# SerCharles/CN-RMA

Hardware: AMD Instinct MI355X
Metric: scenes/sec fwd (40-view->192^3 voxel): dense unprojection + RMA + voxelise + FCAF3D + decode (higher is better)
Workload: dtype f32 (sparse conv f16x3: 22-bit operands, fp32 accumulate; value_f32_conv = exact fp32); 1 GPU; NS: 40 views x 256 ch x 480x640 fp32 maps (channels_last) -> grid 192x192x192, N=300, max_points=500000, FCAF3D MinkResNet34 + head, 1 HIP graph per scene, 3 in flight; M_rows=72216505, M_selected=500000, M_unique=496819

## Files before the change

cn-rma_amd/csrc/rma.hip:

```cpp
#include "common.h"

#include <stdlib.h>

namespace {

struct MarchParams {
  int V, H, W, X, Y, Z, N;
  float vs, ox, oy, oz, t_one, thr;
};

struct Ray {
  float ox, oy, oz, dx, dy, dz;
};

__device__ __forceinline__ Ray make_ray(const float* __restrict__ Pi, float u, float v) {
  float far_[3], o[3];
#pragma unroll
  for (int r = 0; r < 3; ++r) {
    float acc = Pi[r * 4 + 0] * u;
    acc = fmaf(Pi[r * 4 + 1], v, acc);
    acc = fmaf(Pi[r * 4 + 2], 1.0f, acc);
    acc = fmaf(Pi[r * 4 + 3], 1.0f, acc);
    far_[r] = acc;
    o[r] = Pi[r * 4 + 3];
// ... 81 lines not shown
}

template <typename Keep>
__device__ __forceinline__ void neus_march(const Ray& r, const MarchParams& p, const float* __restrict__ tsdf,
                                           float s_out, Keep keep) {
  int a, b;
  if (!clip_steps(r, p, &a, &b)) return;
  double acc = 1.0;
  Sample cur = eval_step(r, a, p, tsdf);
  for (int n = a; n <= b; ++n) {
    Sample nxt;
    if (n + 1 <= b) {
      nxt = eval_step(r, n + 1, p, tsdf);
    } else {
      nxt = cur;
      if (n + 1 <= p.N - 1) { nxt.s = s_out; nxt.valid = false; }
    }
    float alpha = fmaxf((cur.s - nxt.s) / cur.s, 0.0f);
    float T = (float)acc;
    float w = T * alpha;
    if (cur.valid && w >= p.thr) keep(n, cur, w);
    acc *= (double)(1.0f - alpha);
    if ((float)acc < p.thr) break;
    cur = nxt;
  }
}

__device__ __forceinline__ bool ray_setup(const MarchParams& p, const float* __restrict__ proj_inv, int64_t r, Ray* ray,
                                          int* view, int* pix) {
  const int64_t HW = (int64_t)p.H * p.W;
  if (r >= (int64_t)p.V * HW) return false;
  *view = (int)(r / HW);
  *pix = (int)(r - (int64_t)(*view) * HW);
  int v = *pix / p.W, u = *pix - v * p.W;
  *ray = make_ray(proj_inv + (int64_t)(*view) * 16, (float)u, (float)v);
  return true;
}

struct EmitDst {
  float* xyz; int xyz_stride;
  float* w; int w_stride;
  float* feat; int feat_stride;
  int32_t* sample;
  const int32_t* sel;
  const float* w_div;
  float ax, ay, az;
  int64_t sel_cap = 0;
  int64_t out_cap = 0;
};

__global__ __launch_bounds__(256) void neus_count_kernel(MarchParams p, const float* __restrict__ proj_inv,
                                                         const float* __restrict__ tsdf, int32_t* __restrict__ count,
                                                         double* __restrict__ wsum, int2* __restrict__ kept, int cap,
                                                         int32_t* __restrict__ overflow) {
  const int64_t r = (int64_t)blockIdx.x * blockDim.x + threadIdx.x;
  Ray ray; int view, pix;
  if (!ray_setup(p, proj_inv, r, &ray, &view, &pix)) return;
  const float s_out = sigmoid_neg(1.0f);
  int c = 0;
  double ws = 0.0;
  int2* mine = kept ? kept + r * cap : nullptr;
  neus_march(ray, p, tsdf, s_out, [&](int n, const Sample&, float w) {
    if (mine) {
      if (c < cap) mine[c] = make_int2(__float_as_int(w), n);
      else atomicAdd(overflow, 1);
    }
    ++c;
    ws += (double)w;
  });
  count[r] = c;
  wsum[r] = ws;
}

__device__ __forceinline__ float div_by_vs(float a, float vs, float y) {
  float q = a * y;
  float r = fmaf(-vs, q, a);
  q = fmaf(r, y, q);
  r = fmaf(-vs, q, a);
  return fmaf(r, y, q);
}

struct TabSample { float s; bool valid; int rad; };

constexpr int SKIP_B = 4, SKIP_RMAX = 16;

__device__ __forceinline__ TabSample fetch_step(const Ray& r, int n, const MarchParams& p, float inv_vs,
                                                const float* __restrict__ tab, float s_out,
                                                const uint8_t* __restrict__ skip = nullptr, int by = 0, int bz = 0) {
  const float t = (float)n * p.t_one;
  const float x = r.ox + r.dx * t, y = r.oy + r.dy * t, z = r.oz + r.dz * t;
  const float fx = rintf(div_by_vs(x - p.ox, p.vs, inv_vs));
  const float fy = rintf(div_by_vs(y - p.oy, p.vs, inv_vs));
  const float fz = rintf(div_by_vs(z - p.oz, p.vs, inv_vs));
  TabSample o;
  o.valid = (fx >= 0.0f) && (fx < (float)p.X) && (fy >= 0.0f) && (fy < (float)p.Y) && (fz >= 0.0f) && (fz < (float)p.Z);
  o.s = s_out;
  o.rad = 0;
  if (o.valid) {
    o.s = tab[((int)fx * p.Y + (int)fy) * p.Z + (int)fz];
    if (skip != nullptr) o.rad = skip[(((int)fx >> 2) * by + ((int)fy >> 2)) * bz + ((int)fz >> 2)];
  }
  return o;
}

__device__ __forceinline__ void neus_march_block(const MarchParams& p, const float* __restrict__ proj_inv,
                                                 const float* __restrict__ tab, int32_t* __restrict__ count,
                                                 double* __restrict__ wsum, int2* __restrict__ kept, int cap,
                                                 int32_t* __restrict__ overflow, int tiles_x, int tiles_per_view,
                                                 unsigned vblock, const uint8_t* __restrict__ skip = nullptr) {
  int64_t r;
  if (tiles_x > 0) {
    const int view_t = (int)(vblock / (unsigned)tiles_per_view), tile = (int)(vblock - (unsigned)view_t * (unsigned)tiles_per_view);
    const int ty = tile / tiles_x, tx = tile - ty * tiles_x;
    const int w = threadIdx.x >> 6, l = threadIdx.x & 63;
    const int u = tx * 16 + (w & 1) * 8 + (l & 7), v = ty * 16 + (w >> 1) * 8 + (l >> 3);
    if (u >= p.W || v >= p.H) return;
    r = ((int64_t)view_t * p.H + v) * p.W + u;
  } else {
    r = (int64_t)vblock * blockDim.x + threadIdx.x;
  }
  Ray ray; int view, pix;
  if (!ray_setup(p, proj_inv, r, &ray, &view, &pix)) return;
  const float s_out = sigmoid_neg(1.0f);
  const float inv_vs = 1.0f / p.vs;
  int c = 0;
  double ws = 0.0;
  int2* mine = kept + r * cap;
  int a, b;
  if (clip_steps(ray, p, &a, &b)) {
    double acc = 1.0;
    const int by = (p.Y + SKIP_B - 1) / SKIP_B, bz = (p.Z + SKIP_B - 1) / SKIP_B;
    const float m_vox = p.t_one * fmaxf(fmaxf(fabsf(ray.dx), fabsf(ray.dy)), fabsf(ray.dz)) * inv_vs * 1.01f;
    const float per_vox = m_vox > 1e-6f ? 1.0f / m_vox : 0.0f;
    TabSample cur = fetch_step(ray, a, p, inv_vs, tab, s_out, skip, by, bz);
    TabSample n1 = cur, n2 = cur;
    if (a + 1 <= b) n1 = fetch_step(ray, a + 1, p, inv_vs, tab, s_out, skip, by, bz);
    const bool can_skip = p.thr > 0.0f && p.thr <= 1.0f;
    for (int n = a; n <= b; ++n) {
      const bool still = can_skip && (n + 1 <= b) && (n1.s == cur.s);
      if (still && cur.rad > 0) {
        int j = (int)(((float)cur.rad - 1.01f) * per_vox);
        j = min(j, b - 2 - n);
        if (j >= 3) {
          n += j - 1;
          cur.rad = 0;
          n1 = fetch_step(ray, n + 2, p, inv_vs, tab, s_out, skip, by, bz);
          continue;
        }
      }
      if (n + 2 <= b) n2 = fetch_step(ray, n + 2, p, inv_vs, tab, s_out, skip, by, bz);
      if (!still) {
        float s_next;
        if (n + 1 <= b) s_next = n1.s;
        else s_next = (n + 1 <= p.N - 1) ? s_out : cur.s;
        const float alpha = fmaxf((cur.s - s_next) / cur.s, 0.0f);
        const float T = (float)acc;
        const float w = T * alpha;
        if (cur.valid && w >= p.thr) {
          if (c < cap) mine[c] = make_int2(__float_as_int(w), n);
          else atomicAdd(overflow, 1);
          ++c;
          ws += (double)w;
        }
        acc *= (double)(1.0f - alpha);
        if ((float)acc < p.thr) break;
      }
      cur = n1;
      n1 = n2;
    }
  }
  count[r] = c;
  wsum[r] = ws;
}

__global__ __launch_bounds__(256) void neus_march_kernel(MarchParams p, const float* __restrict__ proj_inv,
                                                         const float* __restrict__ tab, int32_t* __restrict__ count,
                                                         double* __restrict__ wsum, int2* __restrict__ kept, int cap,
                                                         int32_t* __restrict__ overflow, int tiles_x, int tiles_per_view,
                                                         const uint8_t* __restrict__ skip) {
  neus_march_block(p, proj_inv, tab, count, wsum, kept, cap, overflow, tiles_x, tiles_per_view, blockIdx.x, skip);
}

__global__ __launch_bounds__(256) void layout_march_kernel(MarchParams p, const float* __restrict__ proj_inv,
                                                           const float* __restrict__ tab, int32_t* __restrict__ count,
                                                           double* __restrict__ wsum, int2* __restrict__ kept, int cap,
                                                           int32_t* __restrict__ overflow, int tiles_x, int tiles_per_view,
                                                           unsigned n_march, unsigned stride,
                                                           const float* __restrict__ src, float* __restrict__ dst, int C,
                                                           int64_t HW, unsigned n_px_tiles, unsigned n_c_blocks,
                                                           const uint8_t* __restrict__ skip) {
  __shared__ float tile[64][65];
  const unsigned b = blockIdx.x;
  if (b % stride == stride - 1 && b / stride < n_march) {
    neus_march_block(p, proj_inv, tab, count, wsum, kept, cap, overflow, tiles_x, tiles_per_view, b / stride, skip);
    return;
  }
  const unsigned before = (b + 1) / stride < n_march ? (b + 1) / stride : n_march;
  const unsigned lb = b - before;
  const int64_t view = lb / (n_px_tiles * n_c_blocks);
  const unsigned rem = lb - (unsigned)view * (n_px_tiles * n_c_blocks);
  const int64_t p0 = (int64_t)(rem % n_px_tiles) * 64;
  const int c0 = (int)(rem / n_px_tiles) * 64;
  const float* sv = src + view * C * HW;
  float* dv = dst + view * C * HW;
  const int q = threadIdx.x & 15, rr = threadIdx.x >> 4;
#pragma unroll
  for (int j = 0; j < 4; ++j) {
    const int c = rr + 16 * j;
    float4 v = make_float4(0.f, 0.f, 0.f, 0.f);
    if (c0 + c < C && p0 + 4 * q < HW) v = *reinterpret_cast<const float4*>(sv + (int64_t)(c0 + c) * HW + p0 + 4 * q);
    tile[c][4 * q + 0] = v.x; tile[c][4 * q + 1] = v.y; tile[c][4 * q + 2] = v.z; tile[c][4 * q + 3] = v.w;
  }
  __syncthreads();
#pragma unroll
  for (int j = 0; j < 4; ++j) {
    const int px = rr + 16 * j;
    if (c0 + 4 * q < C && p0 + px < HW) {
      const float4 o = make_float4(tile[4 * q + 0][px], tile[4 * q + 1][px], tile[4 * q + 2][px], tile[4 * q + 3][px]);
      *reinterpret_cast<float4*>(dv + (p0 + px) * C + c0 + 4 * q) = o;
    }
  }
}

__global__ __launch_bounds__(256) void sigmoid_table_kernel(const float* __restrict__ tsdf, int64_t n, float* __restrict__ tab) {
  for (int64_t i = (int64_t)blockIdx.x * blockDim.x + threadIdx.x; i < n; i += (int64_t)gridDim.x * blockDim.x)
    tab[i] = sigmoid_neg(tsdf[i]);
}

__global__ __launch_bounds__(256) void skip_blockval_kernel(const float* __restrict__ tab, int X, int Y, int Z, int bx, int by, int bz,
                                                            uint32_t* __restrict__ blockval) {
  const int64_t b = (int64_t)blockIdx.x * blockDim.x + threadIdx.x;
  if (b >= (int64_t)bx * by * bz) return;
  const int kz = (int)(b % bz), ky = (int)((b / bz) % by), kx = (int)(b / ((int64_t)bz * by));
  const int x0 = kx * SKIP_B, y0 = ky * SKIP_B, z0 = kz * SKIP_B;
  uint32_t v = 0xFFFFFFFFu;
  if (x0 + SKIP_B <= X && y0 + SKIP_B <= Y && z0 + SKIP_B <= Z) {
    const uint32_t* t = reinterpret_cast<const uint32_t*>(tab);
    v = t[((int64_t)x0 * Y + y0) * Z + z0];
    bool same = true;
    for (int i = 0; i < SKIP_B; ++i)
      for (int j = 0; j < SKIP_B; ++j) {
        const uint32_t* q = t + ((int64_t)(x0 + i) * Y + (y0 + j)) * Z + z0;
#pragma unroll
        for (int k = 0; k < SKIP_B; ++k) same = same && (q[k] == v);
      }
    if (!same) v = 0xFFFFFFFFu;
  }
  blockval[b] = v;
}
__global__ __launch_bounds__(256) void skip_radius_kernel(const uint32_t* __restrict__ blockval, int bx, int by, int bz,
                                                          uint8_t* __restrict__ skip) {
  const int64_t b = (int64_t)blockIdx.x * blockDim.x + threadIdx.x;
  if (b >= (int64_t)bx * by * bz) return;
  const int kz = (int)(b % bz), ky = (int)((b / bz) % by), kx = (int)(b / ((int64_t)bz * by));
  const uint32_t v = blockval[b];
  int r = 0;
  if (v != 0xFFFFFFFFu) {
    constexpr int RB = SKIP_RMAX / SKIP_B;
    for (r = 0; r < RB; ++r) {
      const int d = r + 1;
      if (kx - d < 0 || ky - d < 0 || kz - d < 0 || kx + d >= bx || ky + d >= by || kz + d >= bz) break;
      bool ok = true;
      for (int i = -d; i <= d && ok; ++i)
        for (int j = -d; j <= d && ok; ++j) {
          const bool face = i == -d || i == d || j == -d || j == d;
          const uint32_t* q = blockval + ((int64_t)(kx + i) * by + (ky + j)) * bz + kz;
          if (face) {
            for (int k = -d; k <= d; ++k) ok = ok && q[k] == v;
          } else {
            ok = q[-d] == v && q[d] == v;
          }
        }
      if (!ok) break;
    }
  }
  skip[b] = (uint8_t)(r * SKIP_B);
}

__global__ __launch_bounds__(256) void neus_scatter_records_kernel(int64_t R, const int32_t* __restrict__ row_offset,
                                                                   const int2* __restrict__ kept, int cap,
                                                                   const int32_t* __restrict__ sel, int64_t sel_cap,
                                                                   int64_t rec_cap, int4* __restrict__ rec) {
  const int64_t r = (int64_t)blockIdx.x * blockDim.x + threadIdx.x;
  if (r >= R) return;
  const int64_t m0 = row_offset[r];
  const int c = (int)(row_offset[r + 1] - m0);
  for (int i = 0; i < c; ++i) {
    if (sel && m0 + i >= sel_cap) break;
    const int64_t j = sel ? (int64_t)sel[m0 + i] : m0 + i;
    if (j < 0 || j >= rec_cap) continue;
    const int2 k = kept[r * cap + i];
    rec[j] = make_int4((int)r, k.y, k.x, 0);
  }
}

template <int LPR, int ELEM = 0, typename FT = float>
__global__ __launch_bounds__(256) void neus_emit_rows_kernel(MarchParams p, int C, const float* __restrict__ proj_inv,
                                                            const FT* feat, const FT* const* __restrict__ feat_ref,
                                                            int64_t n_rows, const int32_t* __restrict__ n_rows_dev,
                                                            const int4* __restrict__ rec, EmitDst dst) {
  if (feat_ref != nullptr) feat = *feat_ref;
  const int64_t t = (int64_t)blockIdx.x * blockDim.x + threadIdx.x;
  const int64_t j = t / LPR;
  const int sub = (int)(t % LPR);
  if (j >= live_rows(n_rows, n_rows_dev)) return;
  const int4 rc = rec[j];
  const int64_t r = rc.x;
  const int n = rc.y;
  const float w = __int_as_float(rc.z);
  const int view = (int)(r / ((int64_t)p.H * p.W));
  const int pix = (int)(r - (int64_t)view * p.H * p.W);
  if (sub == 0) {
    const int v = pix / p.W, u = pix - v * p.W;
    const Ray ray = make_ray(proj_inv + (int64_t)view * 16, (float)u, (float)v);
    const float tt = (float)n * p.t_one;
    if (dst.xyz) {
      float* q = dst.xyz + j * dst.xyz_stride;
      q[0] = (ray.ox + ray.dx * tt) + dst.ax;
      q[1] = (ray.oy + ray.dy * tt) + dst.ay;
      q[2] = (ray.oz + ray.dz * tt) + dst.az;
    }
    if (dst.w) dst.w[j * dst.w_stride] = w;
    if (dst.sample) { dst.sample[2 * j] = (int32_t)r; dst.sample[2 * j + 1] = n; }
  }
  if (dst.feat) {
    const FT* f = feat + ((int64_t)view * p.H * p.W + pix) * C;
    float* q = dst.feat + j * dst.feat_stride;
    const bool scaled = dst.w_div != nullptr;
    const float scale = scaled ? w / dst.w_div[0] : 1.0f;
    if constexpr (ELEM == 0) {
      const bool vec = ((C | dst.feat_stride) & 3) == 0 && ((((uintptr_t)dst.feat) | ((uintptr_t)feat)) & 15) == 0;
      if (vec) {
        for (int c = 4 * sub; c < C; c += 4 * LPR) {
          float4 x = *reinterpret_cast<const float4*>(f + c);
          if (scaled) { x.x *= scale; x.y *= scale; x.z *= scale; x.w *= scale; }
          *reinterpret_cast<float4*>(q + c) = x;
        }
      } else {
        for (int c = sub; c < C; c += LPR) q[c] = scaled ? f[c] * scale : f[c];
      }
    } else {
      const bool vec = (C & 7) == 0 && (dst.feat_stride & 3) == 0 && ((((uintptr_t)dst.feat) | ((uintptr_t)feat)) & 15) == 0;
      if (vec) {
        for (int c = 8 * sub; c < C; c += 8 * LPR) {
          float4 x, y;
          elem16_x8<ELEM>(*reinterpret_cast<const uint4*>(f + c), &x, &y);
          if (scaled) { x.x *= scale; x.y *= scale; x.z *= scale; x.w *= scale; y.x *= scale; y.y *= scale; y.z *= scale; y.w *= scale; }
          *reinterpret_cast<float4*>(q + c) = x;
          *reinterpret_cast<float4*>(q + c + 4) = y;
        }
      } else {
        for (int c = sub; c < C; c += LPR) q[c] = scaled ? elem16_to_f32<ELEM>(f[c]) * scale : elem16_to_f32<ELEM>(f[c]);
      }
    }
  }
}

__device__ __forceinline__ void emit_row(const EmitDst& d, int64_t m, float x, float y, float z, float w,
                                         const float* __restrict__ f, int C, int64_t ray, int step) {
// ... 119 lines not shown
                                  float* __restrict__ d) {
  const int64_t HW = (int64_t)H * W;
  const int64_t r = (int64_t)blockIdx.x * blockDim.x + threadIdx.x;
  if (r >= (int64_t)V * HW) return;
  int view = (int)(r / HW);
  int pix = (int)(r - view * HW);
  int v = pix / W, u = pix - v * W;
  Ray ray = make_ray(proj_inv + (int64_t)view * 16, (float)u, (float)v);
  float* dv = d + (int64_t)view * 3 * HW;
  dv[pix] = ray.dx; dv[HW + pix] = ray.dy; dv[2 * HW + pix] = ray.dz;
  if (pix == 0) { o[view * 3] = ray.ox; o[view * 3 + 1] = ray.oy; o[view * 3 + 2] = ray.oz; }
}

__global__ void mean_weight_kernel(const double* __restrict__ wsum_total, const int32_t* __restrict__ m_total,
                                   float* __restrict__ mean_w) {
  mean_w[0] = (float)(wsum_total[0] / (double)m_total[0]);
}

MarchParams make_params(int V, int H, int W, int X, int Y, int Z, float vs, float ox, float oy, float oz, int N,
                        float t_one, float thr) {
  MarchParams p;
  p.V = V; p.H = H; p.W = W; p.X = X; p.Y = Y; p.Z = Z; p.N = N;
  p.vs = vs; p.ox = ox; p.oy = oy; p.oz = oz; p.t_one = t_one; p.thr = thr;
  return p;
}

bool bad_dims(int V, int H, int W, int X, int Y, int Z, int N) {
  return V <= 0 || H <= 0 || W <= 0 || X <= 0 || Y <= 0 || Z <= 0 || N <= 0 ||
         (int64_t)V * H * W >= (int64_t)1 << 31;
}

}

extern "C" int cnrma_ray_params_f32(const float* proj_inv, int V, int H, int W, float* o, float* d, void* stream) {
  if (V <= 0 || H <= 0 || W <= 0) return CNRMA_EINVAL;
  int64_t R = (int64_t)V * H * W;
  hipLaunchKernelGGL(ray_params_kernel, dim3((unsigned)ceil_div(R, 256)), dim3(256), 0, as_stream(stream), proj_inv,
                     V, H, W, o, d);
  CNRMA_LAUNCH_CHECK();
  return 0;
}

extern "C" int cnrma_rma_neus_count_f32(const float* proj_inv, const float* tsdf, int V, int H, int W, int X, int Y,
                                        int Z, float voxel_size, float ox, float oy, float oz, int n_steps,
                                        float t_one, float thr, int32_t* count, double* wsum, void* stream) {
  if (bad_dims(V, H, W, X, Y, Z, n_steps)) return CNRMA_EINVAL;
  MarchParams p = make_params(V, H, W, X, Y, Z, voxel_size, ox, oy, oz, n_steps, t_one, thr);
  int64_t R = (int64_t)V * H * W;
  hipLaunchKernelGGL(neus_count_kernel, dim3((unsigned)ceil_div(R, 256)), dim3(256), 0, as_stream(stream), p,
                     proj_inv, tsdf, count, wsum, (int2*)nullptr, 0, (int32_t*)nullptr);
  CNRMA_LAUNCH_CHECK();
  return 0;
}

#ifdef CNRMA_EXPERIMENTS
__global__ __launch_bounds__(256) void div_check_kernel(const float* __restrict__ a, int64_t n, float vs,
                                                        float* __restrict__ q_fast, float* __restrict__ q_ref) {
  const float y = 1.0f / vs;
  for (int64_t i = (int64_t)blockIdx.x * blockDim.x + threadIdx.x; i < n; i += (int64_t)gridDim.x * blockDim.x) {
    q_fast[i] = div_by_vs(a[i], vs, y);
    q_ref[i] = a[i] / vs;
  }
}

extern "C" int cnrma_debug_div_by_voxel_size_f32(const float* a, int64_t n, float voxel_size, float* q_fast, float* q_ref,
                                                 void* stream) {
  if (n <= 0 || !(voxel_size > 0.0f)) return CNRMA_EINVAL;
  hipLaunchKernelGGL(div_check_kernel, dim3(4096), dim3(256), 0, as_stream(stream), a, n, voxel_size, q_fast, q_ref);
  CNRMA_LAUNCH_CHECK();
  return 0;
}
#endif

extern "C" int cnrma_rma_sigmoid_table_f32(const float* tsdf, int64_t n, float* table, void* stream) {
  if (n <= 0 || tsdf == nullptr || table == nullptr) return CNRMA_EINVAL;
  int64_t blocks = ceil_div(n, 256);
  if (blocks > 4096) blocks = 4096;
  hipLaunchKernelGGL(sigmoid_table_kernel, dim3((unsigned)blocks), dim3(256), 0, as_stream(stream), tsdf, n, table);
  CNRMA_LAUNCH_CHECK();
  return 0;
}

extern "C" size_t cnrma_rma_skip_table_bytes(int X, int Y, int Z) {
  const size_t nb = (size_t)ceil_div(X, SKIP_B) * (size_t)ceil_div(Y, SKIP_B) * (size_t)ceil_div(Z, SKIP_B);
  return ((nb + 255) & ~(size_t)255) + nb * sizeof(uint32_t);
}

extern "C" int cnrma_rma_march_tables_f32(const float* tsdf, int X, int Y, int Z, float* table, void* skip_table, void* stream) {
  if (tsdf == nullptr || table == nullptr || X <= 0 || Y <= 0 || Z <= 0) return CNRMA_EINVAL;
  const int64_t n = (int64_t)X * Y * Z;
  hipStream_t st = as_stream(stream);
  int64_t blocks = ceil_div(n, 256);
  if (blocks > 4096) blocks = 4096;
  hipLaunchKernelGGL(sigmoid_table_kernel, dim3((unsigned)blocks), dim3(256), 0, st, tsdf, n, table);
  if (skip_table != nullptr) {
    const int bx = (int)ceil_div(X, SKIP_B), by = (int)ceil_div(Y, SKIP_B), bz = (int)ceil_div(Z, SKIP_B);
    const int64_t nb = (int64_t)bx * by * bz;
    uint8_t* skip = reinterpret_cast<uint8_t*>(skip_table);
    uint32_t* blockval = reinterpret_cast<uint32_t*>(skip + ((nb + 255) & ~(int64_t)255));
    hipLaunchKernelGGL(skip_blockval_kernel, dim3((unsigned)ceil_div(nb, 256)), dim3(256), 0, st, table, X, Y, Z, bx, by, bz, blockval);
    hipLaunchKernelGGL(skip_radius_kernel, dim3((unsigned)ceil_div(nb, 256)), dim3(256), 0, st, blockval, bx, by, bz, skip);
  }
  CNRMA_LAUNCH_CHECK();
  return 0;
}

static int launch_march(const MarchParams& p, const float* proj_inv, const float* tsdf, const float* sig_table,
                        int32_t* count, double* wsum, void* kept, int cap, int32_t* overflow, const float* feat_nchw,
                        float* feat_nhwc, int C, hipStream_t st, const uint8_t* skip = nullptr) {
  const int64_t R = (int64_t)p.V * p.H * p.W, HW = (int64_t)p.H * p.W;
  hipError_t e = cnrma_fill_bytes(overflow, 0, 4 * sizeof(int32_t), st);
  if (e != hipSuccess) return -(int)e;
  const bool table = sig_table != nullptr && (int64_t)p.X * p.Y * p.Z < ((int64_t)1 << 31);
  const int tx = (int)ceil_div(p.W, 16), ty = (int)ceil_div(p.H, 16);
  const int64_t n_march = (int64_t)p.V * tx * ty;
  if (feat_nchw != nullptr) {
    const int64_t npx = ceil_div(HW, 64), ncb = ceil_div(C, 64), n_layout = npx * ncb * p.V;
    const bool v4 = HW % 4 == 0 && C % 4 == 0 && ((((uintptr_t)feat_nchw) | ((uintptr_t)feat_nhwc)) & 15) == 0;
    if (table && v4 && n_layout + n_march < ((int64_t)1 << 31) && n_layout >= 8 * n_march) {
      unsigned stride = (unsigned)((n_layout + n_march) / n_march);
      if (stride % 2 == 0) --stride;
      hipLaunchKernelGGL(layout_march_kernel, dim3((unsigned)(n_layout + n_march)), dim3(256), 0, st, p, proj_inv, sig_table,
                         count, wsum, reinterpret_cast<int2*>(kept), cap, overflow, tx, tx * ty, (unsigned)n_march, stride,
                         feat_nchw, feat_nhwc, C, HW, (unsigned)npx, (unsigned)ncb, skip);
      CNRMA_LAUNCH_CHECK();
      return 0;
    }
    const int rc = cnrma_nchw_to_nhwc_f32(feat_nchw, feat_nhwc, p.V, C, p.H, p.W, st);
    if (rc != 0) return rc;
  }
  if (table) {
    hipLaunchKernelGGL(neus_march_kernel, dim3((unsigned)n_march), dim3(256), 0, st, p, proj_inv, sig_table, count, wsum,
                       reinterpret_cast<int2*>(kept), cap, overflow, tx, tx * ty, skip);
  } else {
    if (tsdf == nullptr) return CNRMA_EINVAL;
    hipLaunchKernelGGL(neus_count_kernel, dim3((unsigned)ceil_div(R, 256)), dim3(256), 0, st, p, proj_inv, tsdf, count, wsum,
                       reinterpret_cast<int2*>(kept), cap, overflow);
  }
  CNRMA_LAUNCH_CHECK();
  return 0;
}

extern "C" int cnrma_rma_neus_march_f32(const float* proj_inv, const float* tsdf, const float* sig_table, int V, int H,
                                        int W, int X, int Y, int Z, float voxel_size, float ox, float oy, float oz,
                                        int n_steps, float t_one, float thr, int32_t* count, double* wsum, void* kept,
                                        int cap, int32_t* overflow, const void* skip_table, void* stream) {
  if (bad_dims(V, H, W, X, Y, Z, n_steps) || kept == nullptr || cap <= 0 || overflow == nullptr) return CNRMA_EINVAL;
  if (tsdf == nullptr && sig_table == nullptr) return CNRMA_EINVAL;
  MarchParams p = make_params(V, H, W, X, Y, Z, voxel_size, ox, oy, oz, n_steps, t_one, thr);
  return launch_march(p, proj_inv, tsdf, sig_table, count, wsum, kept, cap, overflow, nullptr, nullptr, 0, as_stream(stream),
                      sig_table ? reinterpret_cast<const uint8_t*>(skip_table) : nullptr);
}

extern "C" int cnrma_nchw_to_nhwc_march_f32(const float* feat_nchw, float* feat_nhwc, int C, const float* proj_inv,
                                            const float* tsdf, const float* sig_table, int V, int H, int W, int X, int Y,
                                            int Z, float voxel_size, float ox, float oy, float oz, int n_steps, float t_one,
                                            float thr, int32_t* count, double* wsum, void* kept, int cap, int32_t* overflow,
                                            const void* skip_table, void* stream) {
  if (bad_dims(V, H, W, X, Y, Z, n_steps) || kept == nullptr || cap <= 0 || overflow == nullptr || C <= 0 ||
      feat_nchw == nullptr || feat_nhwc == nullptr)
    return CNRMA_EINVAL;
  if (tsdf == nullptr && sig_table == nullptr) return CNRMA_EINVAL;
  MarchParams p = make_params(V, H, W, X, Y, Z, voxel_size, ox, oy, oz, n_steps, t_one, thr);
  return launch_march(p, proj_inv, tsdf, sig_table, count, wsum, kept, cap, overflow, feat_nchw, feat_nhwc, C, as_stream(stream),
                      sig_table ? reinterpret_cast<const uint8_t*>(skip_table) : nullptr);
}

template <int ELEM = 0, typename FT = float>
static int neus_emit_rows_any(const float* proj_inv, const FT* feat_nhwc, const FT* const* feat_ref, int V, int C, int H, int W,
                                            int n_steps, float t_one, const int32_t* row_offset, int64_t n_out,
                                            const int32_t* n_out_dev, const void* kept, int cap,
                                            const int32_t* sel_index, int64_t sel_cap, void* records,
                                            const float* w_div, float addx, float addy, float addz, float* out_xyz,
                                            int xyz_stride, float* out_w, int w_stride, float* out_feat,
                                            int feat_stride, int32_t* out_sample, void* stream) {
  if (V <= 0 || C <= 0 || H <= 0 || W <= 0 || n_out <= 0 || (kept != nullptr && cap <= 0) || records == nullptr ||
      (kept == nullptr && row_offset != nullptr) || (feat_nhwc == nullptr && feat_ref == nullptr && out_feat != nullptr))
    return CNRMA_EINVAL;
  MarchParams p = make_params(V, H, W, 1, 1, 1, 1.0f, 0.f, 0.f, 0.f, n_steps, t_one, 0.0f);
  EmitDst d{out_xyz, xyz_stride, out_w, w_stride, out_feat, feat_stride, out_sample, nullptr, w_div, addx, addy, addz};
  const int64_t R = (int64_t)V * H * W;
  hipStream_t st = as_stream(stream);
  int4* rec = reinterpret_cast<int4*>(records);
  if (kept != nullptr)
// ... 195 lines not shown
```

cn-rma_amd/csrc/util.hip:

```cpp
#include "common.h"

extern "C" int cnrma_abi_version(void) { return CNRMA_ABI_VERSION; }

extern "C" int cnrma_fill_bytes_u8(void* dst, int byte, size_t n_bytes, void* stream) {
  if (dst == nullptr || (n_bytes & 3) != 0 || (reinterpret_cast<uintptr_t>(dst) & 3) != 0) return CNRMA_EINVAL;
  if (n_bytes == 0) return 0;
  const hipError_t e = cnrma_fill_bytes(dst, byte, n_bytes, reinterpret_cast<hipStream_t>(stream));
  return e == hipSuccess ? 0 : -(int)e;
}

__global__ __launch_bounds__(256) void range_violations_kernel(const int32_t* __restrict__ v, const int32_t* __restrict__ lo,
                                                               const int32_t* __restrict__ hi, int n, int32_t* __restrict__ out) {
  __shared__ int sm[4];
  int c = 0;
  for (int i = threadIdx.x; i < n; i += 256) c += (v[i] < lo[i] || v[i] > hi[i]) ? 1 : 0;
  for (int o = 32; o > 0; o >>= 1) c += __shfl_down(c, o, 64);
  if ((threadIdx.x & 63) == 0) sm[threadIdx.x >> 6] = c;
  __syncthreads();
  if (threadIdx.x == 0) out[0] = sm[0] + sm[1] + sm[2] + sm[3];
}

extern "C" int cnrma_range_violations_i32(const int32_t* values, const int32_t* lo, const int32_t* hi, int n, int32_t* out,
                                          void* stream) {
  if (values == nullptr || lo == nullptr || hi == nullptr || out == nullptr || n <= 0 || n > 4096) return CNRMA_EINVAL;
  hipLaunchKernelGGL(range_violations_kernel, dim3(1), dim3(256), 0, reinterpret_cast<hipStream_t>(stream), values, lo, hi, n, out);
  CNRMA_LAUNCH_CHECK();
  return 0;
}

namespace {

constexpr int SCAN_BLOCK = 256;
constexpr int SCAN_ITEMS = 8;
constexpr int SCAN_TILE = SCAN_BLOCK * SCAN_ITEMS;

template <typename T>
__device__ __forceinline__ int scan_load(const T* in, int64_t i, int64_t n) {
  return i < n ? (int)in[i] : 0;
}

template <typename T>
__global__ __launch_bounds__(SCAN_BLOCK) void scan_tile_sums(const T* __restrict__ in, int32_t* __restrict__ tile_sum,
                                                             int64_t n) {
  __shared__ int smem[SCAN_BLOCK / 64 + 1];
  const int64_t base = (int64_t)blockIdx.x * SCAN_TILE + (int64_t)threadIdx.x * SCAN_ITEMS;
  int s = 0;
#pragma unroll
  for (int j = 0; j < SCAN_ITEMS; ++j) s += scan_load(in, base + j, n);
  int total;
  block_excl_scan<SCAN_BLOCK>(s, smem, &total);
  if (threadIdx.x == 0) tile_sum[blockIdx.x] = total;
}

__global__ __launch_bounds__(1024) void scan_tile_offsets(int32_t* __restrict__ tile_sum, int64_t n_tiles) {
  __shared__ int smem[1024 / 64 + 1];
  const int64_t per = (n_tiles + 1023) / 1024;
  const int64_t lo = (int64_t)threadIdx.x * per;
  const int64_t hi = lo + per < n_tiles ? lo + per : n_tiles;
  int s = 0;
  for (int64_t i = lo; i < hi; ++i) s += tile_sum[i];
  int total;
  int run = block_excl_scan<1024>(s, smem, &total);
  for (int64_t i = lo; i < hi; ++i) {
    const int v = tile_sum[i];
    tile_sum[i] = run;
    run += v;
  }
  if (threadIdx.x == 0) tile_sum[n_tiles] = total;
}

template <typename T, int MODE, bool OWN_OFFSET>
__global__ __launch_bounds__(SCAN_BLOCK) void scan_apply(const T* __restrict__ in, const int32_t* __restrict__ tile_off,
                                                         int32_t* __restrict__ out, int32_t* __restrict__ total_out,
                                                         int64_t n, int64_t n_tiles) {
  __shared__ int smem[SCAN_BLOCK / 64 + 1];
  const int64_t base = (int64_t)blockIdx.x * SCAN_TILE + (int64_t)threadIdx.x * SCAN_ITEMS;
  int v[SCAN_ITEMS];
  int s = 0;
#pragma unroll
  for (int j = 0; j < SCAN_ITEMS; ++j) {
    v[j] = scan_load(in, base + j, n);
    s += v[j];
  }
  int offset, grand = 0;
  if constexpr (OWN_OFFSET) {
    const int upto = blockIdx.x == 0 ? (int)n_tiles : (int)blockIdx.x;
    int part = 0;
    for (int i = threadIdx.x; i < upto; i += SCAN_BLOCK) part += tile_off[i];
    int sum;
    block_excl_scan<SCAN_BLOCK>(part, smem, &sum);
    __syncthreads();
    offset = blockIdx.x == 0 ? 0 : sum;
    grand = sum;
  } else {
    offset = tile_off[blockIdx.x];
    if (blockIdx.x == 0) grand = tile_off[n_tiles];
  }
  int total;
  int run = block_excl_scan<SCAN_BLOCK>(s, smem, &total) + offset;
#pragma unroll
  for (int j = 0; j < SCAN_ITEMS; ++j) {
    if (base + j < n) out[base + j] = (MODE == 0) ? run : (v[j] ? run : -1);
    run += v[j];
  }
  if (blockIdx.x == 0 && threadIdx.x == 0) {
    if (MODE == 0) out[n] = grand;
    if (total_out) total_out[0] = grand;
  }
}

constexpr int SCAN_SINGLE_MAX = 32768;
template <typename T, int MODE>
__global__ __launch_bounds__(1024) void scan_single_kernel(const T* __restrict__ in, int32_t* __restrict__ out,
                                                           int32_t* __restrict__ total_out, int n) {
  __shared__ int smem[1024 / 64 + 1];
  const int per = (n + 1023) / 1024;
  const int lo = threadIdx.x * per, hi = min(lo + per, n);
  int s = 0;
  for (int i = lo; i < hi; ++i) s += (int)in[i];
  int total;
  int run = block_excl_scan<1024>(s, smem, &total);
  for (int i = lo; i < hi; ++i) {
    const int v = (int)in[i];
    out[i] = (MODE == 0) ? run : (v ? run : -1);
    run += v;
  }
  if (threadIdx.x == 0) {
    if (MODE == 0) out[n] = total;
    if (total_out) total_out[0] = total;
  }
}

template <typename T, int MODE>
int run_scan(const T* in, int32_t* out, int32_t* total_out, int64_t n, void* workspace, hipStream_t st) {
  if (n < 0) return CNRMA_EINVAL;
  if (n <= SCAN_SINGLE_MAX) {
    hipLaunchKernelGGL((scan_single_kernel<T, MODE>), dim3(1), dim3(1024), 0, st, in, out, total_out, (int)n);
    CNRMA_LAUNCH_CHECK();
    return 0;
  }
  int64_t n_tiles = ceil_div(n > 0 ? n : 1, SCAN_TILE);
  int32_t* tile = reinterpret_cast<int32_t*>(workspace);
  hipLaunchKernelGGL((scan_tile_sums<T>), dim3((unsigned)n_tiles), dim3(SCAN_BLOCK), 0, st, in, tile, n);
  if (n_tiles <= SCAN_TILE) {
    hipLaunchKernelGGL((scan_apply<T, MODE, true>), dim3((unsigned)n_tiles), dim3(SCAN_BLOCK), 0, st, in, tile, out, total_out,
                       n, n_tiles);
  } else {
    hipLaunchKernelGGL(scan_tile_offsets, dim3(1), dim3(1024), 0, st, tile, n_tiles);
    hipLaunchKernelGGL((scan_apply<T, MODE, false>), dim3((unsigned)n_tiles), dim3(SCAN_BLOCK), 0, st, in, tile, out, total_out,
                       n, n_tiles);
  }
  CNRMA_LAUNCH_CHECK();
  return 0;
}

__global__ __launch_bounds__(256) void sum_f64_partial(const double* __restrict__ in, double* __restrict__ part,
                                                       int64_t n) {
  __shared__ double sm[4];
  double s = 0.0;
  for (int64_t i = (int64_t)blockIdx.x * 256 + threadIdx.x; i < n; i += (int64_t)gridDim.x * 256) s += in[i];
#pragma unroll
  for (int d = 32; d > 0; d >>= 1) s += __shfl_down(s, d, 64);
  if ((threadIdx.x & 63) == 0) sm[threadIdx.x >> 6] = s;
  __syncthreads();
  if (threadIdx.x == 0) part[blockIdx.x] = (sm[0] + sm[1]) + (sm[2] + sm[3]);
}

__global__ __launch_bounds__(256) void sum_f64_final(const double* __restrict__ part, int nparts,
                                                     double* __restrict__ out) {
  __shared__ double sm[4];
  double s = 0.0;
  for (int i = threadIdx.x; i < nparts; i += 256) s += part[i];
#pragma unroll
  for (int d = 32; d > 0; d >>= 1) s += __shfl_down(s, d, 64);
  if ((threadIdx.x & 63) == 0) sm[threadIdx.x >> 6] = s;
  __syncthreads();
  if (threadIdx.x == 0) out[0] = (sm[0] + sm[1]) + (sm[2] + sm[3]);
}

__global__ __launch_bounds__(256) void nchw_to_nhwc_kernel(const float* __restrict__ src, float* __restrict__ dst,
                                                           int C, int64_t HW) {
  __shared__ float tile[32][65];
  const int64_t view = blockIdx.z;
  const int64_t p0 = (int64_t)blockIdx.x * 64;
  const int c0 = blockIdx.y * 32;
  const float* s = src + view * C * HW;
  float* d = dst + view * C * HW;
  const int tx = threadIdx.x & 63, ty = threadIdx.x >> 6;
#pragma unroll
  for (int j = 0; j < 8; ++j) {
    int c = c0 + ty + 4 * j;
    int64_t p = p0 + tx;
    tile[ty + 4 * j][tx] = (c < C && p < HW) ? s[(int64_t)c * HW + p] : 0.0f;
  }
  __syncthreads();
  const int cx = threadIdx.x & 31, py = threadIdx.x >> 5;
#pragma unroll
  for (int j = 0; j < 8; ++j) {
    int c = c0 + cx;
    int64_t p = p0 + py + 8 * j;
    if (c < C && p < HW) d[p * C + c] = tile[cx][py + 8 * j];
  }
}

__global__ __launch_bounds__(256) void nchw_to_nhwc_v4_kernel(const float* __restrict__ src, float* __restrict__ dst, int C,
                                                              int64_t HW) {
  __shared__ float tile[64][65];
  const int64_t view = blockIdx.z;
  const int64_t p0 = (int64_t)blockIdx.x * 64;
  const int c0 = blockIdx.y * 64;
  const float* s = src + view * C * HW;
  float* d = dst + view * C * HW;
  const int q = threadIdx.x & 15, r = threadIdx.x >> 4;
#pragma unroll
  for (int j = 0; j < 4; ++j) {
    const int c = r + 16 * j;
    float4 v = make_float4(0.f, 0.f, 0.f, 0.f);
    if (c0 + c < C && p0 + 4 * q < HW) v = *reinterpret_cast<const float4*>(s + (int64_t)(c0 + c) * HW + p0 + 4 * q);
    tile[c][4 * q + 0] = v.x; tile[c][4 * q + 1] = v.y; tile[c][4 * q + 2] = v.z; tile[c][4 * q + 3] = v.w;
  }
  __syncthreads();
#pragma unroll
  for (int j = 0; j < 4; ++j) {
    const int p = r + 16 * j;
    if (c0 + 4 * q < C && p0 + p < HW) {
      const float4 o = make_float4(tile[4 * q + 0][p], tile[4 * q + 1][p], tile[4 * q + 2][p], tile[4 * q + 3][p]);
      *reinterpret_cast<float4*>(d + (p0 + p) * C + c0 + 4 * q) = o;
    }
  }
}

__global__ __launch_bounds__(256) void nchw_to_nhwc_b16_kernel(const uint16_t* __restrict__ src, uint16_t* __restrict__ dst, int C,
                                                               int64_t HW) {
// ... 473 lines not shown
```

Before: 62.97 scenes/s.

## Use exact distance-field skip table for ray marching and vectorise scan

Replaces the cube-shell radius search with a boundary mask followed by three separable per-axis distance passes. This yields larger empty-space skip radii (up to 252 voxels) that the ray marcher now uses, and the landing logic is reworked so a ray can chain skips without first re-checking the next sample. Separately, the prefix-scan kernels switch to 16 items per thread with int4 vector loads and stores, plus a wave-level scan layout. Risks include wrong skips if the far-distance bound is too loose, and some extra kernel launches and memory for the skip table.

```diff
diff --git a/cn-rma_amd/csrc/rma.hip b/cn-rma_amd/csrc/rma.hip
--- a/cn-rma_amd/csrc/rma.hip
+++ b/cn-rma_amd/csrc/rma.hip
@@ -187,7 +187,17 @@
 
 struct TabSample { float s; bool valid; int rad; };
 
-constexpr int SKIP_B = 4, SKIP_RMAX = 16;
+constexpr int SKIP_B = 4, SKIP_RMAX = 16, SKIP_FAR_MAX = 252;
+#ifndef CNRMA_SKIP_JMIN
+#define CNRMA_SKIP_JMIN 3
+#endif
+constexpr int SKIP_JMIN = CNRMA_SKIP_JMIN;
+
+__host__ __device__ __forceinline__ int64_t skip_align(int64_t n) { return (n + 255) & ~(int64_t)255; }
+__host__ __device__ __forceinline__ int64_t skip_blocks(int X, int Y, int Z) {
+  return (int64_t)((X + SKIP_B - 1) / SKIP_B) * ((Y + SKIP_B - 1) / SKIP_B) * ((Z + SKIP_B - 1) / SKIP_B);
+}
+__host__ __device__ __forceinline__ int64_t skip_far_offset(int64_t nb) { return skip_align(nb) + skip_align(4 * nb); }
 
 __device__ __forceinline__ TabSample fetch_step(const Ray& r, int n, const MarchParams& p, float inv_vs,
                                                 const float* __restrict__ tab, float s_out,
@@ -237,23 +247,29 @@
     const int by = (p.Y + SKIP_B - 1) / SKIP_B, bz = (p.Z + SKIP_B - 1) / SKIP_B;
     const float m_vox = p.t_one * fmaxf(fmaxf(fabsf(ray.dx), fabsf(ray.dy)), fabsf(ray.dz)) * inv_vs * 1.01f;
     const float per_vox = m_vox > 1e-6f ? 1.0f / m_vox : 0.0f;
-    TabSample cur = fetch_step(ray, a, p, inv_vs, tab, s_out, skip, by, bz);
+    const uint8_t* far = skip != nullptr ? skip + skip_far_offset(skip_blocks(p.X, p.Y, p.Z)) : nullptr;
+    TabSample cur = fetch_step(ray, a, p, inv_vs, tab, s_out, far, by, bz);
     TabSample n1 = cur, n2 = cur;
-    if (a + 1 <= b) n1 = fetch_step(ray, a + 1, p, inv_vs, tab, s_out, skip, by, bz);
+    if (a + 1 <= b) n1 = fetch_step(ray, a + 1, p, inv_vs, tab, s_out, far, by, bz);
     const bool can_skip = p.thr > 0.0f && p.thr <= 1.0f;
+    bool landed = false;
     for (int n = a; n <= b; ++n) {
-      const bool still = can_skip && (n + 1 <= b) && (n1.s == cur.s);
-      if (still && cur.rad > 0) {
+      if (can_skip && cur.rad > 0) {
         int j = (int)(((float)cur.rad - 1.01f) * per_vox);
         j = min(j, b - 2 - n);
-        if (j >= 3) {
+        if (j >= SKIP_JMIN && (landed || n1.s == cur.s)) {
           n += j - 1;
-          cur.rad = 0;
-          n1 = fetch_step(ray, n + 2, p, inv_vs, tab, s_out, skip, by, bz);
+          cur = fetch_step(ray, n + 1, p, inv_vs, tab, s_out, far, by, bz);
+          landed = true;
           continue;
         }
       }
-      if (n + 2 <= b) n2 = fetch_step(ray, n + 2, p, inv_vs, tab, s_out, skip, by, bz);
+      if (landed) {
+        n1 = fetch_step(ray, n + 1, p, inv_vs, tab, s_out, far, by, bz);
+        landed = false;
+      }
+      const bool still = can_skip && (n + 1 <= b) && (n1.s == cur.s);
+      if (n + 2 <= b) n2 = fetch_step(ray, n + 2, p, inv_vs, tab, s_out, far, by, bz);
       if (!still) {
         float s_next;
         if (n + 1 <= b) s_next = n1.s;
@@ -353,33 +369,40 @@
   }
   blockval[b] = v;
 }
-__global__ __launch_bounds__(256) void skip_radius_kernel(const uint32_t* __restrict__ blockval, int bx, int by, int bz,
-                                                          uint8_t* __restrict__ skip) {
+__global__ __launch_bounds__(256) void skip_boundary_kernel(const uint32_t* __restrict__ blockval, int bx, int by, int bz,
+                                                            uint8_t* __restrict__ dist) {
   const int64_t b = (int64_t)blockIdx.x * blockDim.x + threadIdx.x;
   if (b >= (int64_t)bx * by * bz) return;
   const int kz = (int)(b % bz), ky = (int)((b / bz) % by), kx = (int)(b / ((int64_t)bz * by));
   const uint32_t v = blockval[b];
-  int r = 0;
-  if (v != 0xFFFFFFFFu) {
-    constexpr int RB = SKIP_RMAX / SKIP_B;
-    for (r = 0; r < RB; ++r) {
-      const int d = r + 1;
-      if (kx - d < 0 || ky - d < 0 || kz - d < 0 || kx + d >= bx || ky + d >= by || kz + d >= bz) break;
-      bool ok = true;
-      for (int i = -d; i <= d && ok; ++i)
-        for (int j = -d; j <= d && ok; ++j) {
-          const bool face = i == -d || i == d || j == -d || j == d;
-          const uint32_t* q = blockval + ((int64_t)(kx + i) * by + (ky + j)) * bz + kz;
-          if (face) {
-            for (int k = -d; k <= d; ++k) ok = ok && q[k] == v;
-          } else {
-            ok = q[-d] == v && q[d] == v;
-          }
-        }
-      if (!ok) break;
-    }
-  }
-  skip[b] = (uint8_t)(r * SKIP_B);
+  bool inner = v != 0xFFFFFFFFu && kx > 0 && ky > 0 && kz > 0 && kx + 1 < bx && ky + 1 < by && kz + 1 < bz;
+  if (inner) {
+    for (int i = -1; i <= 1; ++i)
+      for (int j = -1; j <= 1; ++j) {
+        const uint32_t* q = blockval + ((int64_t)(kx + i) * by + (ky + j)) * bz + kz;
+        inner = inner && q[-1] == v && q[0] == v && q[1] == v;
+      }
+  }
+  dist[b] = inner ? 255 : 0;
+}
+
+__global__ __launch_bounds__(256) void skip_distance_pass_kernel(const uint8_t* __restrict__ in, int64_t nb, int n_axis,
+                                                                 int64_t stride, uint8_t* __restrict__ out,
+                                                                 uint8_t* __restrict__ radii) {
+  const int64_t b = (int64_t)blockIdx.x * blockDim.x + threadIdx.x;
+  if (b >= nb) return;
+  const int k = (int)((b / stride) % n_axis);
+  int best = in[b];
+  for (int d = 1; d < best; ++d) {
+    if (k - d >= 0) best = min(best, max(d, (int)in[b - d * stride]));
+    if (k + d < n_axis) best = min(best, max(d, (int)in[b + d * stride]));
+  }
+  if (radii != nullptr) {
+    out[b] = (uint8_t)min(best * SKIP_B, SKIP_FAR_MAX);
+    radii[b] = (uint8_t)min(best * SKIP_B, SKIP_RMAX);
+  } else {
+    out[b] = (uint8_t)best;
+  }
 }
 
 __global__ __launch_bounds__(256) void neus_scatter_records_kernel(int64_t R, const int32_t* __restrict__ row_offset,
@@ -665,8 +688,8 @@
 }
 
 extern "C" size_t cnrma_rma_skip_table_bytes(int X, int Y, int Z) {
-  const size_t nb = (size_t)ceil_div(X, SKIP_B) * (size_t)ceil_div(Y, SKIP_B) * (size_t)ceil_div(Z, SKIP_B);
-  return ((nb + 255) & ~(size_t)255) + nb * sizeof(uint32_t);
+  const int64_t nb = skip_blocks(X, Y, Z);
+  return (size_t)(skip_far_offset(nb) + 3 * skip_align(nb));
 }
 
 extern "C" int cnrma_rma_march_tables_f32(const float* tsdf, int X, int Y, int Z, float* table, void* skip_table, void* stream) {
@@ -678,11 +701,18 @@
   hipLaunchKernelGGL(sigmoid_table_kernel, dim3((unsigned)blocks), dim3(256), 0, st, tsdf, n, table);
   if (skip_table != nullptr) {
     const int bx = (int)ceil_div(X, SKIP_B), by = (int)ceil_div(Y, SKIP_B), bz = (int)ceil_div(Z, SKIP_B);
-    const int64_t nb = (int64_t)bx * by * bz;
+    const int64_t nb = skip_blocks(X, Y, Z);
     uint8_t* skip = reinterpret_cast<uint8_t*>(skip_table);
-    uint32_t* blockval = reinterpret_cast<uint32_t*>(skip + ((nb + 255) & ~(int64_t)255));
-    hipLaunchKernelGGL(skip_blockval_kernel, dim3((unsigned)ceil_div(nb, 256)), dim3(256), 0, st, table, X, Y, Z, bx, by, bz, blockval);
-    hipLaunchKernelGGL(skip_radius_kernel, dim3((unsigned)ceil_div(nb, 256)), dim3(256), 0, st, blockval, bx, by, bz, skip);
+    uint32_t* blockval = reinterpret_cast<uint32_t*>(skip + skip_align(nb));
+    uint8_t* far = skip + skip_far_offset(nb);
+    uint8_t* d0 = far + skip_align(nb);
+    uint8_t* d1 = d0 + skip_align(nb);
+    const dim3 grid((unsigned)ceil_div(nb, 256)), block(256);
+    hipLaunchKernelGGL(skip_blockval_kernel, grid, block, 0, st, table, X, Y, Z, bx, by, bz, blockval);
+    hipLaunchKernelGGL(skip_boundary_kernel, grid, block, 0, st, blockval, bx, by, bz, d0);
+    hipLaunchKernelGGL(skip_distance_pass_kernel, grid, block, 0, st, d0, nb, bz, (int64_t)1, d1, (uint8_t*)nullptr);
+    hipLaunchKernelGGL(skip_distance_pass_kernel, grid, block, 0, st, d1, nb, by, (int64_t)bz, d0, (uint8_t*)nullptr);
+    hipLaunchKernelGGL(skip_distance_pass_kernel, grid, block, 0, st, d0, nb, bx, (int64_t)by * bz, far, skip);
   }
   CNRMA_LAUNCH_CHECK();
   return 0;
diff --git a/cn-rma_amd/csrc/util.hip b/cn-rma_amd/csrc/util.hip
--- a/cn-rma_amd/csrc/util.hip
+++ b/cn-rma_amd/csrc/util.hip
@@ -31,22 +31,50 @@
 namespace {
 
 constexpr int SCAN_BLOCK = 256;
-constexpr int SCAN_ITEMS = 8;
+constexpr int SCAN_VECS = 4;
+constexpr int SCAN_ITEMS = 4 * SCAN_VECS;
 constexpr int SCAN_TILE = SCAN_BLOCK * SCAN_ITEMS;
+constexpr int SCAN_WAVE_ITEMS = 64 * SCAN_ITEMS;
 
 template <typename T>
 __device__ __forceinline__ int scan_load(const T* in, int64_t i, int64_t n) {
   return i < n ? (int)in[i] : 0;
 }
 
+__device__ __forceinline__ int64_t scan_vec_base(int64_t tile_base, int k) {
+  return tile_base + (int64_t)(threadIdx.x >> 6) * SCAN_WAVE_ITEMS + (int64_t)(k * 64 + (threadIdx.x & 63)) * 4;
+}
+
+template <typename T>
+__device__ __forceinline__ void scan_load_vec(const T* __restrict__ in, int64_t i, int64_t n, bool wide, int v[4]) {
+  static_assert(sizeof(T) == 4 || sizeof(T) == 1, "int32 items or byte masks");
+  if (wide) {
+    if constexpr (sizeof(T) == 4) {
+      const int4 q = *reinterpret_cast<const int4*>(in + i);
+      v[0] = q.x; v[1] = q.y; v[2] = q.z; v[3] = q.w;
+    } else {
+      const uint32_t q = *reinterpret_cast<const uint32_t*>(in + i);
+      v[0] = (int)(q & 255u); v[1] = (int)((q >> 8) & 255u); v[2] = (int)((q >> 16) & 255u); v[3] = (int)(q >> 24);
+    }
+  } else {
+#pragma unroll
+    for (int j = 0; j < 4; ++j) v[j] = scan_load(in, i + j, n);
+  }
+}
+
 template <typename T>
 __global__ __launch_bounds__(SCAN_BLOCK) void scan_tile_sums(const T* __restrict__ in, int32_t* __restrict__ tile_sum,
-                                                             int64_t n) {
+                                                             int64_t n, int aligned) {
   __shared__ int smem[SCAN_BLOCK / 64 + 1];
-  const int64_t base = (int64_t)blockIdx.x * SCAN_TILE + (int64_t)threadIdx.x * SCAN_ITEMS;
+  const int64_t tile_base = (int64_t)blockIdx.x * SCAN_TILE;
+  const bool wide = aligned != 0 && tile_base + SCAN_TILE <= n;
   int s = 0;
 #pragma unroll
-  for (int j = 0; j < SCAN_ITEMS; ++j) s += scan_load(in, base + j, n);
+  for (int k = 0; k < SCAN_VECS; ++k) {
+    int v[4];
+    scan_load_vec(in, scan_vec_base(tile_base, k), n, wide, v);
+    s += (v[0] + v[1]) + (v[2] + v[3]);
+  }
   int total;
   block_excl_scan<SCAN_BLOCK>(s, smem, &total);
   if (threadIdx.x == 0) tile_sum[blockIdx.x] = total;
@@ -72,16 +100,24 @@
 template <typename T, int MODE, bool OWN_OFFSET>
 __global__ __launch_bounds__(SCAN_BLOCK) void scan_apply(const T* __restrict__ in, const int32_t* __restrict__ tile_off,
                                                          int32_t* __restrict__ out, int32_t* __restrict__ total_out,
-                                                         int64_t n, int64_t n_tiles) {
+                                                         int64_t n, int64_t n_tiles, int aligned) {
   __shared__ int smem[SCAN_BLOCK / 64 + 1];
-  const int64_t base = (int64_t)blockIdx.x * SCAN_TILE + (int64_t)threadIdx.x * SCAN_ITEMS;
-  int v[SCAN_ITEMS];
-  int s = 0;
-#pragma unroll
-  for (int j = 0; j < SCAN_ITEMS; ++j) {
-    v[j] = scan_load(in, base + j, n);
-    s += v[j];
-  }
+  __shared__ int wave_sum[SCAN_BLOCK / 64];
+  const int64_t tile_base = (int64_t)blockIdx.x * SCAN_TILE;
+  const bool wide = aligned != 0 && tile_base + SCAN_TILE <= n;
+  const int lane = threadIdx.x & 63, wid = threadIdx.x >> 6;
+  int v[SCAN_VECS][4];
+  int ex[SCAN_VECS];
+  int run = 0;
+#pragma unroll
+  for (int k = 0; k < SCAN_VECS; ++k) {
+    scan_load_vec(in, scan_vec_base(tile_base, k), n, wide, v[k]);
+    const int q = (v[k][0] + v[k][1]) + (v[k][2] + v[k][3]);
+    const int incl = wave_incl_scan(q);
+    ex[k] = run + incl - q;
+    run += __shfl(incl, 63, 64);
+  }
+  if (lane == 0) wave_sum[wid] = run;
   int offset, grand = 0;
   if constexpr (OWN_OFFSET) {
     const int upto = blockIdx.x == 0 ? (int)n_tiles : (int)blockIdx.x;
@@ -89,19 +125,32 @@
     for (int i = threadIdx.x; i < upto; i += SCAN_BLOCK) part += tile_off[i];
     int sum;
     block_excl_scan<SCAN_BLOCK>(part, smem, &sum);
-    __syncthreads();
     offset = blockIdx.x == 0 ? 0 : sum;
     grand = sum;
   } else {
     offset = tile_off[blockIdx.x];
     if (blockIdx.x == 0) grand = tile_off[n_tiles];
-  }
-  int total;
-  int run = block_excl_scan<SCAN_BLOCK>(s, smem, &total) + offset;
-#pragma unroll
-  for (int j = 0; j < SCAN_ITEMS; ++j) {
-    if (base + j < n) out[base + j] = (MODE == 0) ? run : (v[j] ? run : -1);
-    run += v[j];
+    __syncthreads();
+  }
+#pragma unroll
+  for (int w = 0; w < SCAN_BLOCK / 64; ++w) offset += w < wid ? wave_sum[w] : 0;
+#pragma unroll
+  for (int k = 0; k < SCAN_VECS; ++k) {
+    const int64_t i = scan_vec_base(tile_base, k);
+    int r[4];
+    int at = offset + ex[k];
+#pragma unroll
+    for (int j = 0; j < 4; ++j) {
+      r[j] = (MODE == 0) ? at : (v[k][j] ? at : -1);
+      at += v[k][j];
+    }
+    if (wide) {
+      *reinterpret_cast<int4*>(out + i) = make_int4(r[0], r[1], r[2], r[3]);
+    } else {
+#pragma unroll
+      for (int j = 0; j < 4; ++j)
+        if (i + j < n) out[i + j] = r[j];
+    }
   }
   if (blockIdx.x == 0 && threadIdx.x == 0) {
     if (MODE == 0) out[n] = grand;
@@ -141,14 +190,15 @@
   }
   int64_t n_tiles = ceil_div(n > 0 ? n : 1, SCAN_TILE);
   int32_t* tile = reinterpret_cast<int32_t*>(workspace);
-  hipLaunchKernelGGL((scan_tile_sums<T>), dim3((unsigned)n_tiles), dim3(SCAN_BLOCK), 0, st, in, tile, n);
+  const int aligned = (reinterpret_cast<uintptr_t>(out) & 15) == 0 && (reinterpret_cast<uintptr_t>(in) & (4 * sizeof(T) - 1)) == 0;
+  hipLaunchKernelGGL((scan_tile_sums<T>), dim3((unsigned)n_tiles), dim3(SCAN_BLOCK), 0, st, in, tile, n, aligned);
   if (n_tiles <= SCAN_TILE) {
     hipLaunchKernelGGL((scan_apply<T, MODE, true>), dim3((unsigned)n_tiles), dim3(SCAN_BLOCK), 0, st, in, tile, out, total_out,
-                       n, n_tiles);
+                       n, n_tiles, aligned);
   } else {
     hipLaunchKernelGGL(scan_tile_offsets, dim3(1), dim3(1024), 0, st, tile, n_tiles);
     hipLaunchKernelGGL((scan_apply<T, MODE, false>), dim3((unsigned)n_tiles), dim3(SCAN_BLOCK), 0, st, in, tile, out, total_out,
-                       n, n_tiles);
+                       n, n_tiles, aligned);
   }
   CNRMA_LAUNCH_CHECK();
   return 0;
```

Measured after the change: 63.69 scenes/s (median of 6 runs). +1.1%, better.
